# uci-cbcl/RP-Net

Measured on AMD Instinct MI355X. Metric: support/query pairs/sec (fwd+bwd, 1-shot 256x256, T=5), higher is better.
Workload: dtype f32

## Files before the change

rpnet_amd/csrc/conv_split.hip:

```cpp
#include <algorithm>

#include "conv_epilogue.h"
#include "split_bf16.h"

namespace rpnet {

constexpr bool IGLP = true;

template <int NP>
__global__ __launch_bounds__(256) void split_bf16_kernel(const float* __restrict__ x, const float* __restrict__ scale,
                                                          const int mode, unsigned short* __restrict__ out,
                                                          const size_t n8, const FastDiv fC, const size_t plane_elems) {
    RPNET_PASS_PRIORITY();
    for (size_t i = (size_t)blockIdx.x * 256 + threadIdx.x; i < n8; i += (size_t)gridDim.x * 256) {
        const f32x4 a = *reinterpret_cast<const f32x4*>(x + i * 8);
        const f32x4 b = *reinterpret_cast<const f32x4*>(x + i * 8 + 4);
        float v[8] = {a[0], a[1], a[2], a[3], b[0], b[1], b[2], b[3]};
        if (mode) {
            float s = scale[fC.div((unsigned)i)];
            if (mode == 2) s = 1.f - s;
#pragma unroll
            for (int q = 0; q < 8; ++q) v[q] *= s;
        }
        u32x4 o[NP];
        split8<NP>(v, o);
// ... 64 lines not shown
    if ((tid & 63) == 0) red[tid >> 6] = m;
    __syncthreads();
    if (tid == 0) {
        m = fmaxf(fmaxf(red[0], red[1]), fmaxf(red[2], red[3]));
        if (b < cout) t[b] = pow2_scale(m);
        else {
            const int cin = b - cout;
            u[cin < split ? off0 + cin : off1 + (cin - split)] = pow2_scale(m);
        }
    }
}

constexpr int kPackMax = 24;
struct PackItems {
    rpnet_pack_item it[kPackMax];
};

__global__ __launch_bounds__(256) void weight_row_scale_kernel(const PackItems items) {
    const rpnet_pack_item& q = items.it[blockIdx.y];
    if ((int)blockIdx.x >= q.cout + q.cin) return;
    weight_row_scale_block(blockIdx.x, q.w, q.row_scale_wp, q.row_scale_wd, q.cout, q.cin, q.taps, q.cin_off0, q.cin_split, q.cin_off1);
}

template <int NP, bool GATHER>
__device__ __forceinline__ void pack_weight_split_block(float (*tile)[32][33], const int bx, const int by, const float* __restrict__ w,
                                                        unsigned short* __restrict__ wp, unsigned short* __restrict__ wd, int taps,
                                                        int Cin_g, int Cout, int cin_w, int off0, int split, int off1,
                                                        const float* __restrict__ t_row, const float* __restrict__ u_row) {
    const int t = threadIdx.x;
    const int ci0 = bx * 32, co0 = by * 32;
    const int ncin = GATHER ? 32 : min(32, cin_w - ci0);
    if (GATHER) {
        for (int e = t; e < 32 * 32 * taps; e += 256) {
            const int col = e / (32 * taps), r = e - col * (32 * taps);
            const int c = r / taps, tap = r - c * taps;
            const int R = ci0 + c;
            int src = -1;
            if (R >= off0 && R < off0 + split) src = R - off0;
            else if (R >= off1 && R < off1 + (cin_w - split)) src = split + (R - off1);
            tile[tap][c][col] = src >= 0 ? w[((size_t)(co0 + col) * cin_w + src) * taps + tap] : 0.f;
        }
    } else {
        const int nel = ncin * taps;
        for (int e = t; e < 32 * nel; e += 256) {
            const int col = e / nel, r = e - col * nel;
            const int c = r / taps, tap = r - c * taps;
            tile[tap][c][col] = w[((size_t)(co0 + col) * cin_w + ci0) * taps + r];
        }
    }
    __syncthreads();
    const size_t plane = (size_t)taps * Cin_g * Cout;
    for (int e = t; e < taps * 32 * 4; e += 256) {
        const int g = e & 3, cl = (e >> 2) & 31, tap = e >> 7;
        if (g * 8 < ncin) {
            const int cin = ci0 + g * 8;
            const int row = GATHER ? cin : (cin < split ? off0 + cin : off1 + (cin - split));
            float v[8];
#pragma unroll
            for (int q = 0; q < 8; ++q) v[q] = tile[tap][g * 8 + q][cl];
            if (NP <= 2) {
                const float inv = 1.f / t_row[co0 + cl];
#pragma unroll
                for (int q = 0; q < 8; ++q) v[q] *= inv;
            }
            u32x4 o[NP];
            split8<NP>(v, o);
            const size_t dst = (((size_t)tap * (Cin_g >> 5) + (row >> 5)) * Cout + co0 + cl) * 32 + (row & 31);
#pragma unroll
            for (int p = 0; p < NP; ++p) *reinterpret_cast<u32x4*>(wp + p * plane + dst) = o[p];
        }
    }
    if (wd) {
        for (int e = t; e < taps * 32 * 4; e += 256) {
            const int g = e & 3, c = (e >> 2) & 31, tap = e >> 7;
            if (c < ncin) {
                const int cin = ci0 + c;
                const int row = GATHER ? cin : (cin < split ? off0 + cin : off1 + (cin - split));
                float v[8];
#pragma unroll
                for (int q = 0; q < 8; ++q) v[q] = tile[tap][c][g * 8 + q];
                if (NP <= 2) {
                    const float inv = 1.f / u_row[row];
#pragma unroll
                    for (int q = 0; q < 8; ++q) v[q] *= inv;
                }
                u32x4 o[NP];
                split8<NP>(v, o);
                const int tf = taps - 1 - tap;
                const size_t dst = (((size_t)tf * (Cout >> 5) + (co0 >> 5)) * Cin_g + row) * 32 + g * 8;
#pragma unroll
                for (int p = 0; p < NP; ++p) *reinterpret_cast<u32x4*>(wd + p * plane + dst) = o[p];
            }
        }
    }
}

__host__ __device__ static inline bool pack_needs_gather(const rpnet_pack_item& q) {
    return (q.cin % 8) || (q.cin_off0 % 8) || (q.cin_split % 8) || (q.cin_off1 % 8);
}

template <int NP>
__global__ __launch_bounds__(256) void pack_weight_split_kernel(const PackItems items) {
    __shared__ float tile[9][32][33];
    const rpnet_pack_item& q = items.it[blockIdx.y];
    const bool gather = pack_needs_gather(q);
    const int tx = gather ? q.cin_pad / 32 : (q.cin + 31) / 32, ntiles = tx * (q.cout / 32);
    if ((int)blockIdx.x >= ntiles) return;
    if (gather)
        pack_weight_split_block<NP, true>(tile, blockIdx.x % tx, blockIdx.x / tx, q.w, (unsigned short*)q.wp, (unsigned short*)q.wd, q.taps,
                                          q.cin_pad, q.cout, q.cin, q.cin_off0, q.cin_split, q.cin_off1, q.row_scale_wp, q.row_scale_wd);
    else
        pack_weight_split_block<NP, false>(tile, blockIdx.x % tx, blockIdx.x / tx, q.w, (unsigned short*)q.wp, (unsigned short*)q.wd, q.taps,
                                           q.cin_pad, q.cout, q.cin, q.cin_off0, q.cin_split, q.cin_off1, q.row_scale_wp, q.row_scale_wd);
}

template <int WGM, int WM, int WN, int NP, bool DB>
__global__ __launch_bounds__(WGM * 128, (DB ? 1 : (WGM == 2 ? 2 : 1))) void conv_igemm_split_kernel(
    const rpnet_conv_desc d, const int M, const int Cin, const int Cout, const int tiles_n, const int ntiles) {
    constexpr int NT = WGM * 128;
    constexpr int BM = 32 * WGM * WM, BN = 64 * WN;
    constexpr int RP = NT / 4;
    constexpr int AJ = BM / RP, BJ = (BN + RP - 1) / RP;
    constexpr bool B_PART = BN < RP;
    constexpr int A_BYTES = BM * 64, B_BYTES = BN * 64;
    constexpr int STAGE = NP * (A_BYTES + B_BYTES);
    __shared__ __attribute__((aligned(16))) unsigned char smem[cmax((DB ? 2 : 1) * STAGE, epilogue_lds_bytes<WN, WGM>())];

    const int t = threadIdx.x;
    const int lane = t & 63, wv = t >> 6;
    const int li = lane & 31, h = lane >> 5;
    const int wm = wv >> 1, wn = wv & 1;

    const int tile = xcd_swizzle(blockIdx.x, ntiles);
    const int tm = tile / tiles_n, tn = tile - tm * tiles_n;
    const int m0 = tm * BM, n0 = tn * BN;

// ... 805 lines not shown
                      "pack_conv_weights_split: channel ranges exceed cin_pad (item %d)", i);
        pk.it[i] = q;
        max_rows = std::max(max_rows, q.cout + q.cin);
        max_tiles = std::max(max_tiles, (pack_needs_gather(q) ? q.cin_pad / 32 : cdiv(q.cin, 32)) * (q.cout / 32));
    }
    for (int i = n; i < kPackMax; ++i) pk.it[i] = items[0];
    hipStream_t s = (hipStream_t)stream;
    if (planes <= 2)
        hipLaunchKernelGGL(weight_row_scale_kernel, dim3(max_rows, n), dim3(256), 0, s, pk);
    if (planes == 3) hipLaunchKernelGGL(pack_weight_split_kernel<3>, dim3(max_tiles, n), dim3(256), 0, s, pk);
    else if (planes == 2) hipLaunchKernelGGL(pack_weight_split_kernel<2>, dim3(max_tiles, n), dim3(256), 0, s, pk);
    else hipLaunchKernelGGL(pack_weight_split_kernel<1>, dim3(max_tiles, n), dim3(256), 0, s, pk);
    return check_launch("pack_conv_weights_split");
}

extern "C" int rpnet_pack_conv_weight_split(const float* w, void* wp, void* wd, int cout, int cin, int taps, int cin_off0,
                                            int cin_split, int cin_off1, int cin_pad, int planes, float* row_scale_wp,
                                            float* row_scale_wd, rpnet_stream_t stream) {
    rpnet_pack_item q;
    q.w = w; q.wp = wp; q.wd = wd; q.row_scale_wp = row_scale_wp; q.row_scale_wd = row_scale_wd;
    q.cout = cout; q.cin = cin; q.taps = taps; q.cin_off0 = cin_off0; q.cin_split = cin_split; q.cin_off1 = cin_off1; q.cin_pad = cin_pad;
    return rpnet_pack_conv_weights_split(&q, 1, planes, stream);
}
```

rpnet_amd/csrc/conv_up4_dma.hip:

```cpp
#include <type_traits>

#include "conv_epilogue.h"
#include "lds_dma.h"
#include "split_bf16.h"

namespace rpnet {

template <int N, int I = 0, typename F>
__device__ __forceinline__ void static_for_u(F&& f) {
    if constexpr (I < N) {
        f(std::integral_constant<int, I>{});
        static_for_u<N, I + 1>(f);
    }
}

template <int N>
__device__ __forceinline__ void wait_vmcnt() {
    static_assert(N >= 0 && N < 64, "vmcnt is a 6-bit counter");
    asm volatile("s_waitcnt vmcnt(%0)" ::"n"(N) : "memory");
}

template <int TW>
struct PatchRowsUp {
    static constexpr bool kAlwaysValid = true;
// ... 225 lines not shown
    asm volatile("s_waitcnt vmcnt(0)" ::: "memory");
    __builtin_amdgcn_s_barrier();

    if constexpr (DG) {
        conv_epilogue<WM, WN, 2, PatchRows<TW>, false>(d, acc, PatchRows<TW>{(n * Hl + y0) * Wl + x0, Wl}, d.N * Hl * Wl, Ncols, Hl * Wl, n0, tm,
                                                        wm, wn, li, h, smem);
    } else {
        conv_epilogue<WM, WN, 2, PatchRowsUp<TW>, false>(d, acc, PatchRowsUp<TW>{(n * H + 2 * y0 + fpy) * W + 2 * x0 + fpx, 2 * W}, d.N * H * W,
                                                          Cout_out, H * W, n0 - fphase * Cout_out, tm * 4 + fphase, wm, wn, li, h, smem,
                                                          fphase * Cout_out);
    }
}

__global__ __launch_bounds__(256) void upconv_collapse_kernel(const float* __restrict__ w, float* __restrict__ wc, const int Cout, const int Cin) {
    const size_t i = (size_t)blockIdx.x * 256 + threadIdx.x;
    if (i >= (size_t)4 * Cout * Cin) return;
    const int ci = (int)(i % Cin);
    const int co = (int)((i / Cin) % Cout), ph = (int)(i / ((size_t)Cin * Cout));
    const int py = ph >> 1, px = ph & 1;
    float k[9];
#pragma unroll
    for (int q = 0; q < 9; ++q) k[q] = w[((size_t)co * Cin + ci) * 9 + q];
    float o[4];
#pragma unroll
    for (int r = 0; r < 2; ++r)
#pragma unroll
        for (int c = 0; c < 2; ++c) {
            const int ya = r == 0 ? 0 : (py ? 2 : 1), yb = r == 0 ? (py ? 1 : 0) : 2;
            const int xa = c == 0 ? 0 : (px ? 2 : 1), xb = c == 0 ? (px ? 1 : 0) : 2;
            float s = 0.f;
            for (int ky = ya; ky <= yb; ++ky)
                for (int kx = xa; kx <= xb; ++kx) s += k[ky * 3 + kx];
            o[r * 2 + c] = s;
        }
    *reinterpret_cast<f32x4*>(wc + i * 4) = f32x4{o[0], o[1], o[2], o[3]};
}

static int up4_tw(int Hl, int Wl) {
    if (Wl % 32 == 0 && Hl % 8 == 0) return 32;
    if (Wl % 16 == 0 && Hl % 16 == 0) return 16;
    return 0;
}

static int up4_plan(const rpnet_conv_desc* d, int mode, int* tw, int* Kc, int* Ncols) {
    if (!d || (d->split_planes != 2 && d->split_planes != 1) || d->H % 2 || d->W % 2 || d->C1 || d->Co1 || d->x1 || d->y1) return 0;
    const int Hl = d->H / 2, Wl = d->W / 2;
    const bool one = d->split_planes == 1;
    *tw = up4_tw(Hl, Wl);
    if (!*tw || d->C0 % (one ? 64 : 32) || d->Co0 % (one ? 128 : 64)) return 0;
    *Kc = mode == 1 ? d->C0 : 4 * d->C0;
    *Ncols = mode == 1 ? 4 * d->Co0 : d->Co0;
    const size_t lim = (size_t)1 << 31;
    const size_t src = (size_t)d->N * (mode == 1 ? Hl * Wl : d->H * d->W) * d->C0 * 2 * d->split_planes;
    if (src >= lim || (size_t)2 * 4 * *Kc * *Ncols * 2 >= lim || (size_t)d->N * d->H * d->W >= lim) return 0;
    const long tiles_m = (long)d->N * Hl * Wl / 256;
    if (mode == 1) return (d->Co0 % 128 == 0) ? 2 : 1;
    if (one) return 2;
// ... 54 lines not shown
```

rpnet_amd/csrc/split_bf16.h:

```cpp
#pragma once
#include "common.h"

namespace rpnet {

using bf16x8 = __attribute__((ext_vector_type(8))) __bf16;
using u32x4 = __attribute__((ext_vector_type(4))) unsigned;
using u32x2 = __attribute__((ext_vector_type(2))) unsigned;

__device__ __forceinline__ unsigned bf16_bits(float x) {
    return (unsigned)__builtin_bit_cast(unsigned short, (__bf16)x);
}
__device__ __forceinline__ float bf16_val(unsigned b) { return __uint_as_float(b << 16); }

__device__ __forceinline__ unsigned f16_bits(float x) {
    return (unsigned)__builtin_bit_cast(unsigned short, (_Float16)x);
}
__device__ __forceinline__ float f16_val(unsigned b) {
    return (float)__builtin_bit_cast(_Float16, (unsigned short)b);
}

__device__ __forceinline__ float pow2_scale(float b) {
    const unsigned u = __float_as_uint(fmaxf(b, 0.f));
    int e = (int)((u >> 23) & 255u) - 127 + ((u & 0x7fffffu) ? 1 : 0);
    e = e - 15;
    e = e < -100 ? -100 : (e > 100 ? 100 : e);
    return __uint_as_float((unsigned)(e + 127) << 23);
}

template <int NP>
__device__ __forceinline__ void split8(const float (&v)[8], u32x4 (&out)[NP]) {
    unsigned hb[8], mb[8], lb[8];
#pragma unroll
    for (int q = 0; q < 8; ++q) {
        if (NP <= 2) {
            hb[q] = f16_bits(v[q]);
            if (NP == 2) mb[q] = f16_bits(v[q] - f16_val(hb[q]));
            continue;
        }
        hb[q] = bf16_bits(v[q]);
        const float r1 = v[q] - bf16_val(hb[q]);
        mb[q] = bf16_bits(r1);
        if (NP > 2) lb[q] = bf16_bits(r1 - bf16_val(mb[q]));
    }
#pragma unroll
    for (int q = 0; q < 4; ++q) {
        out[0][q] = hb[2 * q] | (hb[2 * q + 1] << 16);
        if (NP > 1) out[NP > 1 ? 1 : 0][q] = mb[2 * q] | (mb[2 * q + 1] << 16);
        if (NP > 2) out[NP - 1][q] = lb[2 * q] | (lb[2 * q + 1] << 16);
    }
// ... 21 lines not shown
```

rpnet_amd/functional.py:

```python
import collections
import contextlib
import ctypes as C
import os

import torch
from torch.autograd import Function
from torch.autograd.function import once_differentiable

from . import hip
from .hip import ConvDesc, call, ptr, query

BN_EPS = 1e-5
BN_MOMENTUM = 0.1

_ASYNC = {"on": False, "side": {}, "pending": set(), "queued": False, "fifo": [], "keep": []}

_MODES = {"f32": (0, False, 0), "bf16x3": (3, False, 0), "f16x2": (3, True, 2), "f16": (3, True, 1)}
_CORR_PRED_PLANES = True
_MATH = {}


def set_conv_math(mode):
    _MATH["mode"] = mode
    _MATH["planes"], _MATH["f16"], _MATH["f16_planes"] = _MODES[mode]
# ... 484 lines not shown
        if self._wp is None:
            self._pack_f32()
        return self._wd

    def split_packs(self, planes):
        pk = self.wps.get(planes) if self.wps else None
        if pk is None:
            w = self._weight
            pk = self.alloc_split(planes)
            call("rpnet_pack_conv_weight_split", ptr(w), ptr(pk[0]), ptr(pk[1]), self.cout, self.cin, self.taps,
                 self.off0, self.split, self.off1, self.cin_pad, planes, ptr(pk[2]) if planes <= 2 else None,
                 ptr(pk[3]) if planes <= 2 else None)
        return pk

    def up4_packs(self, planes):
        up = getattr(self, "_up4", None)
        if up is None:
            up = self._up4 = {}
        pk = up.get(planes)
        if pk is None:
            w = self._weight
            wc = torch.empty((4 * self.cout, self.cin, 2, 2), device=w.device, dtype=torch.float32)
            call("rpnet_upconv_collapse_weights", ptr(w), ptr(wc), self.cout, self.cin)
            n = 4 * self.cin * 4 * self.cout
            wp4 = torch.empty((planes, n), device=w.device, dtype=torch.float16)
            wd4 = torch.empty((planes, n), device=w.device, dtype=torch.float16)
            t4 = torch.empty(4 * self.cout, device=w.device, dtype=torch.float32)
            u4 = torch.empty(self.cin, device=w.device, dtype=torch.float32)
            call("rpnet_pack_conv_weight_split", ptr(wc), ptr(wp4), ptr(wd4), 4 * self.cout, self.cin, 4, 0, self.cin, self.cin, self.cin,
                 planes, ptr(t4), ptr(u4))
            pk = up[planes] = (wp4, wd4, t4, u4)
        return pk

    def alloc_split(self, planes):
        if self.wps is None:
            self.wps = {}
        n = self.taps * self.cin_pad * self.cout
        padded = self.cin_pad != self.cin
        w = self._weight
        key = (w.data_ptr(), tuple(w.shape), planes, self.cin_pad, self.off0, self.split, self.off1, str(w.device))
        if padded and self._pool is not None and key in self._pool:
            pk = self._pool[key]
            self.wps[planes] = pk
            return pk
        mk = torch.zeros if padded else torch.empty
        dt = torch.bfloat16 if planes == 3 else torch.float16
        wps, wds = mk((planes, n), device=w.device, dtype=dt), mk((planes, n), device=w.device, dtype=dt)
        if planes == 3:
            pk = (wps, wds)
        else:
            t = torch.empty(self.cout, device=w.device, dtype=torch.float32)
            u = (torch.ones if padded else torch.empty)(self.cin_pad, device=w.device, dtype=torch.float32)
            pk = (wps, wds, t, u)
        if padded and self._pool is not None:
            self._pool[key] = pk
        self.wps[planes] = pk
        return pk


class WeightCache:

    def __init__(self):
        self._d = {}
        self._ready = None
        self._padded = {}

    def clear(self):
        self._d.clear()
        self._ready = None

    def prepack_async(self, weights, planes, device, up4=()):
        main = torch.cuda.current_stream(device)
        ps = _pack_stream(device)
        ps.wait_stream(main)
        self._ready = None
        with torch.cuda.stream(ps):
            self.prepack(weights, planes, up4)
            ev = torch.cuda.Event()
            ev.record(ps)
        self._ready = (ev, set(), torch.cuda.is_current_stream_capturing())

    def get(self, weight, split=None):
        if self._ready is not None and self._ready[2] and not torch.cuda.is_current_stream_capturing():
            self._ready = None
        if self._ready is not None:
            sid = hip.stream()
            if sid not in self._ready[1]:
                torch.cuda.current_stream(weight.device).wait_event(self._ready[0])
                self._ready[1].add(sid)
        key = (weight.data_ptr(), weight._version, None if split is None else tuple(split))
        pw = self._d.get(key)
        if pw is None:
            pw = PackedWeight(weight.detach(), split, self._padded)
            self._d[key] = pw
        return pw

    def prepack(self, weights, planes, up4=()):
        up4 = list(up4) if (_UP4 and planes in (1, 2)) else []
        if up4:
            skip = {id(w) for w in up4}
            weights = [w for w in weights if id(w) not in skip]
            for w in up4:
                self.get(w).up4_packs(planes)
        pws = [self.get(w) for w in weights]
        pws = [pw for pw in pws if pw.taps == 9 and pw.cin_pad == pw.cin and pw.cin % 32 == 0 and pw.cout % 32 == 0
               and not (pw.wps and planes in pw.wps)]
        for i in range(0, len(pws), hip.PACK_MAX):
            chunk = pws[i:i + hip.PACK_MAX]
            items = (hip.PackItem * len(chunk))()
            for it, pw in zip(items, chunk):
                bufs = pw.alloc_split(planes)
                it.w, it.wp, it.wd = ptr(pw._weight), ptr(bufs[0]), ptr(bufs[1])
                it.row_scale_wp, it.row_scale_wd = (ptr(bufs[2]), ptr(bufs[3])) if planes <= 2 else (None, None)
                it.cout, it.cin, it.taps = pw.cout, pw.cin, pw.taps
                it.cin_off0, it.cin_split, it.cin_off1, it.cin_pad = pw.off0, pw.split, pw.off1, pw.cin_pad
            call("rpnet_pack_conv_weights_split", items, len(chunk), planes)

    def materialize(self, weights, planes):
        for w in weights:
            pw = self.get(w)
            if planes and pw.taps == 9 and pw.cin_pad == pw.cin and pw.cin % 32 == 0 and pw.cout % 32 == 0:
# ... 1101 lines not shown
```

rpnet_amd/hip.py:

```python
import ctypes as C
import os

import torch

_LIB_PATH = os.environ.get("RPNET_LIB_PATH") or os.path.join(os.path.dirname(os.path.abspath(__file__)), "librpnet_hip.so")
_lib = None

vp, ci, cf, cs, cd = C.c_void_p, C.c_int, C.c_float, C.c_size_t, C.c_double


class ConvDesc(C.Structure):
    _fields_ = [("x0", vp), ("x1", vp), ("C0", ci), ("C1", ci), ("w", vp), ("bias", vp), ("in_scale", vp),
                ("in_scale_mode", ci), ("y0", vp), ("y1", vp), ("Co0", ci), ("Co1", ci), ("ep_scale", vp),
                ("ep_shift", vp), ("ep_relu", ci), ("out_scale", vp), ("out_scale_mode", ci), ("accumulate", ci),
                ("N", ci), ("H", ci), ("W", ci), ("taps", ci), ("upsample", ci), ("groups", ci), ("dilation", ci), ("stats_partial", vp), ("split_planes", ci), ("y_split", vp), ("split_out_planes", ci),
                ("acc_scale_col", vp), ("acc_scale_x", vp), ("acc_scale_dy", vp), ("bnb_y", vp), ("bnb_stats", vp), ("bnb_partial", vp), ("bnb_pmax", vp), ("bnb_groups", ci),
                ("acc_scale_x1", vp), ("out_absmax", vp), ("tune", ci), ("y_split_scale", vp), ("splitk_ws", vp), ("splitk_ws_bytes", cs),
                ("skip_mask", vp), ("skip_mode", ci), ("skip_halo", ci), ("skip_ws", vp), ("tile_skip", vp),
                ("y_enc", vp), ("y_enc_stride", ci)]


PACK_MAX = 24


# ... 127 lines not shown
    "rpnet_adam_step_guarded": (ci, [vp, C.c_int64, vp, vp, vp, vp, vp, vp, vp, vp]),
}
GUARD_ABI_SYMBOLS = tuple(_GUARD_SIGS)
GUARD_ABI_VERSION = 1

_SURFACE_SIGS = {
    "rpnet_surface_abi_version": (ci, []),
    "rpnet_surface_workspace_bytes": (cs, [ci, ci, ci]),
    "rpnet_surface_tally": (ci, [vp, ci, vp, ci, ci, ci, ci, ci, vp, C.c_int64, vp, C.c_int64, C.c_int64, vp, cs, vp]),
}
SURFACE_ABI_SYMBOLS = tuple(_SURFACE_SIGS)
SURFACE_ABI_VERSION = 1

_CC_SIGS = {
    "rpnet_cc_abi_version": (ci, []),
    "rpnet_cc_workspace_bytes": (cs, [ci, ci, ci]),
    "rpnet_cc_label": (ci, [vp, ci, ci, ci, ci, ci, ci, vp, vp, C.c_int64, C.c_int64, vp, cs, vp]),
    "rpnet_cc_keep_largest": (ci, [vp, ci, vp, ci, ci, ci, ci, ci, vp, ci, vp, C.c_int64, vp, C.c_int64, C.c_int64, vp, cs, vp]),
}
CC_ABI_SYMBOLS = tuple(_CC_SIGS)
CC_ABI_VERSION = 1


def lib_path():
    return _LIB_PATH


def load():
    global _lib
    if _lib is None:
        if not os.path.exists(_LIB_PATH):
            raise RuntimeError(f"{_LIB_PATH} not found: build it with `make -C rpnet_amd/csrc` "
                               "(or __graft_entry__.build()); rpnet_amd has no CPU fallback")
        lib = C.CDLL(_LIB_PATH)
        lib.rpnet_version.restype = ci
        if lib.rpnet_version() != ABI_VERSION:
            raise RuntimeError(f"{_LIB_PATH} has ABI version {lib.rpnet_version()}, this binding was written for {ABI_VERSION} "
                               "(include/rpnet_abi.h RPNET_ABI_VERSION): rebuild it with `make -C rpnet_amd/csrc`")
        for name, (res, args) in (list(_SIGS.items()) + list(_EVAL_SIGS.items()) + list(_OPTIM_SIGS.items()) + list(_GUARD_SIGS.items())
                                  + list(_SURFACE_SIGS.items()) + list(_CC_SIGS.items())):
            fn = getattr(lib, name, None)
            if fn is None:
                raise RuntimeError(f"{_LIB_PATH} does not export {name}: rebuild it with `make -C rpnet_amd/csrc`")
            fn.restype, fn.argtypes = res, args
        if lib.rpnet_eval_abi_version() != EVAL_ABI_VERSION:
            raise RuntimeError(f"{_LIB_PATH} has evaluation-item ABI version {lib.rpnet_eval_abi_version()}, this binding was written for "
                               f"{EVAL_ABI_VERSION} (include/rpnet_eval_abi.h): rebuild it with `make -C rpnet_amd/csrc`")
        if lib.rpnet_optim_abi_version() != OPTIM_ABI_VERSION:
            raise RuntimeError(f"{_LIB_PATH} has optimizer ABI version {lib.rpnet_optim_abi_version()}, this binding was written for "
                               f"{OPTIM_ABI_VERSION} (include/rpnet_optim_abi.h): rebuild it with `make -C rpnet_amd/csrc`")
        if lib.rpnet_guard_abi_version() != GUARD_ABI_VERSION:
            raise RuntimeError(f"{_LIB_PATH} has gradient-guard ABI version {lib.rpnet_guard_abi_version()}, this binding was written for "
                               f"{GUARD_ABI_VERSION} (include/rpnet_guard_abi.h): rebuild it with `make -C rpnet_amd/csrc`")
        if lib.rpnet_surface_abi_version() != SURFACE_ABI_VERSION:
            raise RuntimeError(f"{_LIB_PATH} has surface-distance ABI version {lib.rpnet_surface_abi_version()}, this binding was written "
                               f"for {SURFACE_ABI_VERSION} (include/rpnet_surface_abi.h): rebuild it with `make -C rpnet_amd/csrc`")
        if lib.rpnet_cc_abi_version() != CC_ABI_VERSION:
            raise RuntimeError(f"{_LIB_PATH} has connected-component ABI version {lib.rpnet_cc_abi_version()}, this binding was written "
                               f"for {CC_ABI_VERSION} (include/rpnet_cc_abi.h): rebuild it with `make -C rpnet_amd/csrc`")
        _lib = lib
    return _lib


def ptr(t):
    return None if t is None else t.data_ptr()


try:
    _raw_stream, _cur_device = torch._C._cuda_getCurrentRawStream, torch._C._cuda_getDevice
except AttributeError:
    _raw_stream = None


def stream():
    if _raw_stream is not None:
        return _raw_stream(_cur_device())
    return torch.cuda.current_stream().cuda_stream


def call(name, *args):
    lib = load()
    rc = getattr(lib, name)(*args, stream())
# ... 14 lines not shown
```

rpnet_amd/modules.py:

```python
import itertools
import os

import torch
import torch.nn as nn

from . import functional as RF
from .schedule import Schedule

_FANIN = 2
_PREPACK = True
_ZSKIP = True
_F16_MIN_PIXELS = int(os.environ.get("RPNET_F16_MIN_PIXELS", "262144"))
_F16_MIN_PIXELS_EVAL = int(os.environ.get("RPNET_F16_MIN_PIXELS_EVAL", "524288"))
_CRE_STREAMS = True
_CRE_STREAMS_MAX_PIXELS = 16384
_CRE_STREAMS_TRAIN = os.environ.get("RPNET_CRE_STREAMS_TRAIN", "1") == "1"
_ENC_STREAMS = int(os.environ.get("RPNET_ENC_STREAMS", "1"))
_NET_SERIAL = itertools.count(1)


def _to_nhwc(x):
    return x.permute(0, 2, 3, 1).contiguous()


# ... 352 lines not shown
        if repack:
            cache.clear()

        supp = (supp_imgs[0][0] if n_ways * n_shots == 1 else torch.cat([torch.cat(way, 0) for way in supp_imgs], 0)).float()
        qry = qry_imgs[0].float()
        RF.hip.require_gpu(supp, qry)
        ns = supp.shape[0]
        f16_min, f16_min_eval = sch.get("f16_min_pixels", _F16_MIN_PIXELS), sch.get("f16_min_pixels_eval", _F16_MIN_PIXELS_EVAL)
        thr = f16_min if (self.training or not f16_min_eval or not f16_min or RF._EVAL_PREDICT) else f16_min_eval
        RF.set_f16_active((ns + B) * H * W >= thr)
        pred_key = None
        if RF.f16_mode():
            RF.reset_absmax_pool(supp.device)
            if not self.training and not torch.is_grad_enabled() and RF._EVAL_PREDICT:
                pred_key = (self._serial, RF.conv_math(), ns, B, H, W, self.num_iter, n_ways, n_shots, self.forced_masks is not None)
                RF.pred_begin(supp.device, pred_key, allow=not getattr(self, "_pred_redo", False))
        planes = RF.pack_planes()
        if _PREPACK and planes and repack:
            ups = ()
            if self.training or RF.f16_mode():
                enc_n = (ns + B,) if ns == B else (ns, B)
                ups = tuple(m.up[1].weight for m, f in ((self.encoder.Up5, 8), (self.encoder.Up4, 4))
                            if RF.up4_layer_ok(m.up[1].weight, planes, [(n, H // f, W // f) for n in enc_n + ((ns, B) if ns == B else ())]))
            if self.training and supp.is_cuda:
                cache.prepack_async(self._pack_weights(), planes, supp.device, ups)
            else:
                cache.prepack(self._pack_weights(), planes, ups)
        enc_mask = fore_mask[0][0].float() if self.encoder.mask_feature_map else None
        if enc_mask is not None and ns != B:
            raise NotImplementedError("mask_feature_map with more than one support image per episode: the reference "
                                      "concatenates B masks onto Wa*Sh*B images (net/unet.py:438) and fails")
        enc_streams, fanin = sch.get("enc_streams", _ENC_STREAMS), sch.get("fanin", _FANIN)
        two_chains = (self.training and supp.is_cuda and enc_mask is None and
                      (enc_streams == 2 or (enc_streams == 1 and ns != B and ns <= 2 * B)))
        RF.order_begin(two_chains)
        split_fan = False
        if ns == B and not two_chains:
            d4 = self.encoder.forward_nhwc(torch.cat([supp, qry], 0).reshape(ns + B, H, W, 1), cache, groups=2,
                                           mask=None if enc_mask is None else torch.cat([enc_mask, enc_mask], 0))
            s_supp = s_qry = d4.scale
            d4 = d4.x
            split_fan = d4.requires_grad and fanin >= 2 and n_ways * n_shots == 1
            if split_fan:
                uses = RF.SplitFan.apply(d4, ns, 2, 2 * self.num_iter)
                supp_d4, qry_d4, fan_supp, fan_qry = uses[0], uses[2], uses[:2], uses[2:]
            else:
                supp_d4, qry_d4 = RF.SplitRows.apply(d4, ns) if (d4.requires_grad and fanin) else (d4[:ns], d4[ns:])
        elif two_chains:
            main, side = torch.cuda.current_stream(supp.device), RF._cre_stream(supp.device)
            qin = qry.reshape(B, H, W, 1)
# ... 153 lines not shown
```

Baseline: 486.1.

## Fuse per-layer weight packing into one table-driven two-kernel launch

Replaces the per-layer weight row-scale and split-pack launches with a precomputed device tile table covering every layer, including collapsed up-convolutions and the padded correlation layer. Two kernels run over it: one computes row and column maxima with atomics into double-buffered scratch, the other packs and publishes the scales. The goal is to cut the many small kernel launches and host calls made each training step during prepack. It also adds a vectorized quad load for 9-tap tiles. In exchange it brings a new ABI, plan caching keyed on weight pointers, and ping-pong scale buffers whose correctness depends on kernel ordering.

```diff
diff --git a/include/rpnet_pack_abi.h b/include/rpnet_pack_abi.h
--- /dev/null
+++ b/include/rpnet_pack_abi.h
@@ -0,0 +1,41 @@
+#ifndef RPNET_PACK_ABI_H
+#define RPNET_PACK_ABI_H
+
+#include <stddef.h>
+#include <stdint.h>
+
+#include "rpnet_abi.h"
+
+#ifdef __cplusplus
+extern "C" {
+#endif
+
+#define RPNET_PACK_ABI_VERSION 1
+int rpnet_pack_abi_version(void);
+
+struct rpnet_pack_layer {
+    rpnet_pack_item item;
+    float* maxima;
+    int32_t collapse;
+    int32_t reserved;
+};
+
+struct rpnet_pack_tile {
+    int32_t layer;
+    uint16_t bx, by;
+};
+
+struct rpnet_pack_head {
+    int32_t n_layers, n_tiles;
+    uint32_t set_scale;
+    uint32_t set_pack;
+};
+
+size_t rpnet_pack_plan_bytes(const struct rpnet_pack_layer* layers, int n);
+int rpnet_pack_plan(const struct rpnet_pack_layer* layers, int n, int planes, void* table, size_t table_bytes, int* n_tiles);
+int rpnet_pack_fused(void* table, int n_layers, int n_tiles, int planes, rpnet_stream_t stream);
+
+#ifdef __cplusplus
+}
+#endif
+#endif
diff --git a/rpnet_amd/csrc/conv_split.hip b/rpnet_amd/csrc/conv_split.hip
--- a/rpnet_amd/csrc/conv_split.hip
+++ b/rpnet_amd/csrc/conv_split.hip
@@ -1,6 +1,7 @@
 #include <algorithm>
 
 #include "conv_epilogue.h"
+#include "rpnet_pack_abi.h"
 #include "split_bf16.h"
 
 namespace rpnet {
@@ -111,14 +112,22 @@
     weight_row_scale_block(blockIdx.x, q.w, q.row_scale_wp, q.row_scale_wd, q.cout, q.cin, q.taps, q.cin_off0, q.cin_split, q.cin_off1);
 }
 
-template <int NP, bool GATHER>
-__device__ __forceinline__ void pack_weight_split_block(float (*tile)[32][33], const int bx, const int by, const float* __restrict__ w,
-                                                        unsigned short* __restrict__ wp, unsigned short* __restrict__ wd, int taps,
-                                                        int Cin_g, int Cout, int cin_w, int off0, int split, int off1,
-                                                        const float* __restrict__ t_row, const float* __restrict__ u_row) {
+template <bool GATHER, bool QUADS = false>
+__device__ __forceinline__ int pack_tile_load(float (*tile)[32][33], const int ci0, const int co0, const float* __restrict__ w, int taps,
+                                              int cin_w, int off0, int split, int off1) {
     const int t = threadIdx.x;
-    const int ci0 = bx * 32, co0 = by * 32;
     const int ncin = GATHER ? 32 : min(32, cin_w - ci0);
+    if (QUADS && !GATHER && taps == 9 && ncin == 32 && cin_w % 4 == 0 && (reinterpret_cast<size_t>(w) & 15) == 0) {
+#pragma unroll
+        for (int j = 0; j < 9; ++j) {
+            const int e = t + 256 * j;
+            const int col = e / 72, r = (e - col * 72) * 4;
+            const f32x4 v = *reinterpret_cast<const f32x4*>(w + ((size_t)(co0 + col) * cin_w + ci0) * 9 + r);
+#pragma unroll
+            for (int i = 0; i < 4; ++i) tile[(r + i) % 9][(r + i) / 9][col] = v[i];
+        }
+        return ncin;
+    }
     if (GATHER) {
         for (int e = t; e < 32 * 32 * taps; e += 256) {
             const int col = e / (32 * taps), r = e - col * (32 * taps);
@@ -137,18 +146,30 @@
             tile[tap][c][col] = w[((size_t)(co0 + col) * cin_w + ci0) * taps + r];
         }
     }
-    __syncthreads();
+    return ncin;
+}
+
+template <bool GATHER>
+__device__ __forceinline__ int pack_row(const int cin, int off0, int split, int off1) {
+    return GATHER ? cin : (cin < split ? off0 + cin : off1 + (cin - split));
+}
+
+template <int NP, bool GATHER, bool FROM_MAX = false>
+__device__ __forceinline__ void pack_tile_store(float (*tile)[32][33], const int ci0, const int co0, const int ncin,
+                                                unsigned short* __restrict__ wp, unsigned short* __restrict__ wd, int taps, int Cin_g,
+                                                int Cout, int off0, int split, int off1, const float* __restrict__ t_row,
+                                                const float* __restrict__ u_row) {
+    const int t = threadIdx.x;
     const size_t plane = (size_t)taps * Cin_g * Cout;
     for (int e = t; e < taps * 32 * 4; e += 256) {
         const int g = e & 3, cl = (e >> 2) & 31, tap = e >> 7;
         if (g * 8 < ncin) {
-            const int cin = ci0 + g * 8;
-            const int row = GATHER ? cin : (cin < split ? off0 + cin : off1 + (cin - split));
+            const int row = pack_row<GATHER>(ci0 + g * 8, off0, split, off1);
             float v[8];
 #pragma unroll
             for (int q = 0; q < 8; ++q) v[q] = tile[tap][g * 8 + q][cl];
             if (NP <= 2) {
-                const float inv = 1.f / t_row[co0 + cl];
+                const float inv = 1.f / (FROM_MAX ? pow2_scale(t_row[co0 + cl]) : t_row[co0 + cl]);
 #pragma unroll
                 for (int q = 0; q < 8; ++q) v[q] *= inv;
             }
@@ -163,13 +184,12 @@
         for (int e = t; e < taps * 32 * 4; e += 256) {
             const int g = e & 3, c = (e >> 2) & 31, tap = e >> 7;
             if (c < ncin) {
-                const int cin = ci0 + c;
-                const int row = GATHER ? cin : (cin < split ? off0 + cin : off1 + (cin - split));
+                const int row = pack_row<GATHER>(ci0 + c, off0, split, off1);
                 float v[8];
 #pragma unroll
                 for (int q = 0; q < 8; ++q) v[q] = tile[tap][c][g * 8 + q];
                 if (NP <= 2) {
-                    const float inv = 1.f / u_row[row];
+                    const float inv = 1.f / (FROM_MAX ? pow2_scale(u_row[row]) : u_row[row]);
 #pragma unroll
                     for (int q = 0; q < 8; ++q) v[q] *= inv;
                 }
@@ -182,6 +202,16 @@
             }
         }
     }
+}
+
+template <int NP, bool GATHER>
+__device__ __forceinline__ void pack_weight_split_block(float (*tile)[32][33], const int bx, const int by, const float* __restrict__ w,
+                                                        unsigned short* __restrict__ wp, unsigned short* __restrict__ wd, int taps,
+                                                        int Cin_g, int Cout, int cin_w, int off0, int split, int off1,
+                                                        const float* __restrict__ t_row, const float* __restrict__ u_row) {
+    const int ncin = pack_tile_load<GATHER>(tile, bx * 32, by * 32, w, taps, cin_w, off0, split, off1);
+    __syncthreads();
+    pack_tile_store<NP, GATHER>(tile, bx * 32, by * 32, ncin, wp, wd, taps, Cin_g, Cout, off0, split, off1, t_row, u_row);
 }
 
 __host__ __device__ static inline bool pack_needs_gather(const rpnet_pack_item& q) {
@@ -201,6 +231,161 @@
     else
         pack_weight_split_block<NP, false>(tile, blockIdx.x % tx, blockIdx.x / tx, q.w, (unsigned short*)q.wp, (unsigned short*)q.wd, q.taps,
                                            q.cin_pad, q.cout, q.cin, q.cin_off0, q.cin_split, q.cin_off1, q.row_scale_wp, q.row_scale_wd);
+}
+
+struct PackWork {
+    const rpnet_pack_layer* L;
+    int bx, by;
+};
+__device__ __forceinline__ PackWork pack_work(const void* table) {
+    const rpnet_pack_head* h = (const rpnet_pack_head*)table;
+    const rpnet_pack_layer* layers = (const rpnet_pack_layer*)(h + 1);
+    const rpnet_pack_tile tl = ((const rpnet_pack_tile*)(layers + h->n_layers))[blockIdx.x];
+    return PackWork{layers + tl.layer, (int)tl.bx, (int)tl.by};
+}
+
+__device__ __forceinline__ void collapse_tile_load(float (&k)[4][9], const int ci0, const int co0, const float* __restrict__ w, int cin_w) {
+#pragma unroll
+    for (int j = 0; j < 4; ++j) {
+        const int pr = threadIdx.x + 256 * j, col = pr >> 5, c = pr & 31;
+        const float* src = w + ((size_t)(co0 + col) * cin_w + ci0 + c) * 9;
+#pragma unroll
+        for (int q = 0; q < 9; ++q) k[j][q] = src[q];
+    }
+}
+__device__ __forceinline__ void collapse_tile_phase(float (*tile)[32][33], const float (&k)[4][9], const int ph) {
+#pragma unroll
+    for (int j = 0; j < 4; ++j) {
+        const int pr = threadIdx.x + 256 * j, col = pr >> 5, c = pr & 31;
+        float o[4];
+        upconv_collapse_taps(k[j], ph >> 1, ph & 1, o);
+#pragma unroll
+        for (int q = 0; q < 4; ++q) tile[q][c][col] = o[q];
+    }
+}
+
+__device__ __forceinline__ void pack_tile_maxima(float (*tile)[32][33], unsigned* smax, const int taps, const int ncin) {
+    const int t = threadIdx.x;
+    if (t < 64) smax[t] = 0u;
+    __syncthreads();
+    const int idx = t & 31, part = (t >> 5) & 3;
+    float m = 0.f;
+    if (t < 128) {
+        for (int tap = 0; tap < taps; ++tap)
+            for (int c = part; c < ncin; c += 4) m = fmaxf(m, fabsf(tile[tap][c][idx]));
+    } else if (idx < ncin) {
+        for (int j = part; j < taps * 32; j += 4) m = fmaxf(m, fabsf(tile[j >> 5][idx][j & 31]));
+    }
+    atomicMax(&smax[(t < 128 ? 0 : 32) + idx], __float_as_uint(m));
+    __syncthreads();
+}
+
+template <bool GATHER>
+__device__ __forceinline__ void pack_maxima_merge(const unsigned* smax, float* mx, const rpnet_pack_item& q, const int ci0, const int row0,
+                                                  const int ncin) {
+    const int t = threadIdx.x;
+    if (t < 32) atomicMax((unsigned*)mx + row0 + t, smax[t]);
+    else if (t < 64 && t - 32 < ncin) {
+        const int cin = ci0 + t - 32;
+        const bool real = !GATHER || (cin >= q.cin_off0 && cin < q.cin_off0 + q.cin_split) ||
+                          (cin >= q.cin_off1 && cin < q.cin_off1 + (q.cin - q.cin_split));
+        if (real) atomicMax((unsigned*)mx + q.cout + pack_row<GATHER>(cin, q.cin_off0, q.cin_split, q.cin_off1), smax[t]);
+    }
+}
+
+__global__ __launch_bounds__(256) void pack_fused_scale_kernel(void* table) {
+    __shared__ float tile[9][32][33];
+    __shared__ unsigned smax[64];
+    rpnet_pack_head* h = (rpnet_pack_head*)table;
+    const unsigned set = h->set_scale & 1u;
+    if (blockIdx.x == 0 && threadIdx.x == 0) h->set_pack = set ^ 1u;
+    const PackWork k = pack_work(table);
+    const rpnet_pack_item& q = k.L->item;
+    float* mx = k.L->maxima + (size_t)set * (q.cout + q.cin_pad);
+    const int ci0 = k.bx * 32, co0 = k.by * 32;
+    if (k.L->collapse) {
+        float k9[4][9];
+        collapse_tile_load(k9, ci0, co0, q.w, q.cin);
+        for (int ph = 0; ph < 4; ++ph) {
+            if (ph) __syncthreads();
+            collapse_tile_phase(tile, k9, ph);
+            pack_tile_maxima(tile, smax, 4, 32);
+            pack_maxima_merge<false>(smax, mx, q, ci0, ph * (q.cout >> 2) + co0, 32);
+        }
+    } else if (pack_needs_gather(q)) {
+        const int ncin = pack_tile_load<true>(tile, ci0, co0, q.w, q.taps, q.cin, q.cin_off0, q.cin_split, q.cin_off1);
+        pack_tile_maxima(tile, smax, q.taps, ncin);
+        pack_maxima_merge<true>(smax, mx, q, ci0, co0, ncin);
+    } else {
+        const int ncin = pack_tile_load<false, true>(tile, ci0, co0, q.w, q.taps, q.cin, q.cin_off0, q.cin_split, q.cin_off1);
+        pack_tile_maxima(tile, smax, q.taps, ncin);
+        pack_maxima_merge<false>(smax, mx, q, ci0, co0, ncin);
+    }
+}
+
+template <bool GATHER>
+__device__ __forceinline__ void pack_scales_publish(const rpnet_pack_item& q, const float* mx, float* other, const int bx, const int ci0,
+                                                    const int row0, const bool cols) {
+    const int t = threadIdx.x;
+    if (bx == 0 && t < 32) {
+        q.row_scale_wp[row0 + t] = pow2_scale(mx[row0 + t]);
+        other[row0 + t] = 0.f;
+    }
+    if (cols && t >= 32 && t < 64) {
+        const int cin = ci0 + t - 32;
+        const bool real = GATHER ? ((cin >= q.cin_off0 && cin < q.cin_off0 + q.cin_split) ||
+                                    (cin >= q.cin_off1 && cin < q.cin_off1 + (q.cin - q.cin_split)))
+                                 : cin < q.cin;
+        if (real) {
+            const int row = pack_row<GATHER>(cin, q.cin_off0, q.cin_split, q.cin_off1);
+            q.row_scale_wd[row] = pow2_scale(mx[q.cout + row]);
+            other[q.cout + row] = 0.f;
+        }
+    }
+}
+
+template <int NP>
+__global__ __launch_bounds__(256) void pack_fused_kernel(void* table) {
+    __shared__ float tile[9][32][33];
+    constexpr bool F16 = NP <= 2;
+    rpnet_pack_head* h = (rpnet_pack_head*)table;
+    const PackWork k = pack_work(table);
+    const rpnet_pack_item& q = k.L->item;
+    const float* mx = nullptr;
+    float* other = nullptr;
+    if (F16) {
+        const unsigned clr = h->set_pack & 1u;
+        if (blockIdx.x == 0 && threadIdx.x == 0) h->set_scale = clr;
+        mx = k.L->maxima + (size_t)(clr ^ 1u) * (q.cout + q.cin_pad);
+        other = k.L->maxima + (size_t)clr * (q.cout + q.cin_pad);
+    }
+    const int ci0 = k.bx * 32, co0 = k.by * 32;
+    unsigned short* wp = (unsigned short*)q.wp;
+    unsigned short* wd = (unsigned short*)q.wd;
+    if (k.L->collapse) {
+        float k9[4][9];
+        collapse_tile_load(k9, ci0, co0, q.w, q.cin);
+        for (int ph = 0; ph < 4; ++ph) {
+            const int row0 = ph * (q.cout >> 2) + co0;
+            if (ph) __syncthreads();
+            collapse_tile_phase(tile, k9, ph);
+            __syncthreads();
+            pack_tile_store<NP, false, true>(tile, ci0, row0, 32, wp, wd, 4, q.cin_pad, q.cout, 0, q.cin, q.cin, mx, mx + q.cout);
+            if (F16) pack_scales_publish<false>(q, mx, other, k.bx, ci0, row0, k.by == 0 && ph == 0);
+        }
+    } else if (pack_needs_gather(q)) {
+        const int ncin = pack_tile_load<true>(tile, ci0, co0, q.w, q.taps, q.cin, q.cin_off0, q.cin_split, q.cin_off1);
+        __syncthreads();
+        pack_tile_store<NP, true, true>(tile, ci0, co0, ncin, wp, wd, q.taps, q.cin_pad, q.cout, q.cin_off0, q.cin_split, q.cin_off1, mx,
+                                        mx + q.cout);
+        if (F16) pack_scales_publish<true>(q, mx, other, k.bx, ci0, co0, k.by == 0);
+    } else {
+        const int ncin = pack_tile_load<false, true>(tile, ci0, co0, q.w, q.taps, q.cin, q.cin_off0, q.cin_split, q.cin_off1);
+        __syncthreads();
+        pack_tile_store<NP, false, true>(tile, ci0, co0, ncin, wp, wd, q.taps, q.cin_pad, q.cout, q.cin_off0, q.cin_split, q.cin_off1, mx,
+                                         mx + q.cout);
+        if (F16) pack_scales_publish<false>(q, mx, other, k.bx, ci0, co0, k.by == 0);
+    }
 }
 
 template <int WGM, int WM, int WN, int NP, bool DB>
@@ -1052,3 +1237,83 @@
     q.cout = cout; q.cin = cin; q.taps = taps; q.cin_off0 = cin_off0; q.cin_split = cin_split; q.cin_off1 = cin_off1; q.cin_pad = cin_pad;
     return rpnet_pack_conv_weights_split(&q, 1, planes, stream);
 }
+
+extern "C" int rpnet_pack_abi_version(void) { return RPNET_PACK_ABI_VERSION; }
+
+namespace rpnet {
+static int pack_layer_tiles(const rpnet_pack_layer& l, int* tx, int* ty) {
+    const rpnet_pack_item& q = l.item;
+    *tx = l.collapse ? q.cin / 32 : (pack_needs_gather(q) ? q.cin_pad / 32 : cdiv(q.cin, 32));
+    *ty = (l.collapse ? q.cout / 4 : q.cout) / 32;
+    return *tx * *ty;
+}
+
+static int pack_plan_check(const rpnet_pack_layer* layers, int n, int planes, long* tiles) {
+    RPNET_REQUIRE(layers && n >= 1, RPNET_ERR_ARG, "pack_plan: %d layers", n);
+    RPNET_REQUIRE(planes >= 0 && planes <= 3, RPNET_ERR_SHAPE, "pack_plan: planes %d", planes);
+    *tiles = 0;
+    for (int i = 0; i < n; ++i) {
+        const rpnet_pack_item& q = layers[i].item;
+        RPNET_REQUIRE(q.w && q.wp, RPNET_ERR_ARG, "pack_plan: null pointer (layer %d)", i);
+        RPNET_REQUIRE(planes == 0 || planes == 3 || (q.row_scale_wp && q.row_scale_wd && layers[i].maxima), RPNET_ERR_ARG,
+                      "pack_plan: fp16 planes (1 or 2) need the row scale outputs and the maxima (layer %d)", i);
+        RPNET_REQUIRE(q.cout > 0 && q.cin > 0 && q.cout % 32 == 0 && q.cin_pad > 0 && q.cin_pad % 32 == 0 &&
+                          (q.taps == 9 || q.taps == 1 || q.taps == 4),
+                      RPNET_ERR_SHAPE, "pack_plan: cout %d cin %d cin_pad %d taps %d (layer %d)", q.cout, q.cin, q.cin_pad, q.taps, i);
+        RPNET_REQUIRE(q.cin_off0 >= 0 && q.cin_off1 >= 0 && q.cin_split >= 0 && q.cin_split <= q.cin &&
+                          q.cin_off0 + q.cin_split <= q.cin_pad && q.cin_off1 + (q.cin - q.cin_split) <= q.cin_pad,
+                      RPNET_ERR_SHAPE, "pack_plan: channel ranges exceed cin_pad (layer %d)", i);
+        if (layers[i].collapse)
+            RPNET_REQUIRE(q.taps == 4 && q.cout % 128 == 0 && q.cin % 32 == 0 && q.cin_off0 == 0 && q.cin_split == q.cin &&
+                              q.cin_off1 == q.cin && q.cin_pad == q.cin,
+                          RPNET_ERR_SHAPE, "pack_plan: collapsed layer %d: cout %d cin %d taps %d, or channel ranges", i, q.cout, q.cin, q.taps);
+        int tx, ty;
+        *tiles += pack_layer_tiles(layers[i], &tx, &ty);
+        RPNET_REQUIRE(tx <= 65535 && ty <= 65535 && *tiles < (1l << 30), RPNET_ERR_SHAPE, "pack_plan: too many tiles (layer %d)", i);
+    }
+    return RPNET_OK;
+}
+}
+
+extern "C" size_t rpnet_pack_plan_bytes(const rpnet_pack_layer* layers, int n) {
+    long tiles = 0;
+    if (rpnet::pack_plan_check(layers, n, 0, &tiles) != RPNET_OK) return 0;
+    return sizeof(rpnet_pack_head) + (size_t)n * sizeof(rpnet_pack_layer) + (size_t)tiles * sizeof(rpnet_pack_tile);
+}
+
+extern "C" int rpnet_pack_plan(const rpnet_pack_layer* layers, int n, int planes, void* table, size_t table_bytes, int* n_tiles) {
+    using namespace rpnet;
+    RPNET_REQUIRE(table && n_tiles, RPNET_ERR_ARG, "pack_plan: null pointer");
+    RPNET_REQUIRE(planes >= 1, RPNET_ERR_SHAPE, "pack_plan: planes %d", planes);
+    long tiles = 0;
+    const int rc = pack_plan_check(layers, n, planes, &tiles);
+    if (rc != RPNET_OK) return rc;
+    const size_t need = sizeof(rpnet_pack_head) + (size_t)n * sizeof(rpnet_pack_layer) + (size_t)tiles * sizeof(rpnet_pack_tile);
+    RPNET_REQUIRE(table_bytes >= need, RPNET_ERR_WORKSPACE, "pack_plan: table of %zu bytes, %zu needed", table_bytes, need);
+    rpnet_pack_head* h = (rpnet_pack_head*)table;
+    *h = rpnet_pack_head{n, (int)tiles, 0u, 1u};
+    rpnet_pack_layer* L = (rpnet_pack_layer*)(h + 1);
+    rpnet_pack_tile* T = (rpnet_pack_tile*)(L + n);
+    for (int i = 0; i < n; ++i) {
+        L[i] = layers[i];
+        L[i].reserved = 0;
+        int tx, ty;
+        pack_layer_tiles(layers[i], &tx, &ty);
+        for (int by = 0; by < ty; ++by)
+            for (int bx = 0; bx < tx; ++bx) *T++ = rpnet_pack_tile{i, (uint16_t)bx, (uint16_t)by};
+    }
+    *n_tiles = (int)tiles;
+    return RPNET_OK;
+}
+
+extern "C" int rpnet_pack_fused(void* table, int n_layers, int n_tiles, int planes, rpnet_stream_t stream) {
+    using namespace rpnet;
+    RPNET_REQUIRE(table && n_layers >= 1 && n_tiles >= 1, RPNET_ERR_ARG, "pack_fused: table %p, %d layers, %d tiles", table, n_layers, n_tiles);
+    RPNET_REQUIRE(planes >= 1 && planes <= 3, RPNET_ERR_SHAPE, "pack_fused: planes %d", planes);
+    hipStream_t s = (hipStream_t)stream;
+    if (planes <= 2) hipLaunchKernelGGL(pack_fused_scale_kernel, dim3(n_tiles), dim3(256), 0, s, table);
+    if (planes == 3) hipLaunchKernelGGL(pack_fused_kernel<3>, dim3(n_tiles), dim3(256), 0, s, table);
+    else if (planes == 2) hipLaunchKernelGGL(pack_fused_kernel<2>, dim3(n_tiles), dim3(256), 0, s, table);
+    else hipLaunchKernelGGL(pack_fused_kernel<1>, dim3(n_tiles), dim3(256), 0, s, table);
+    return check_launch("pack_fused");
+}
diff --git a/rpnet_amd/csrc/conv_up4_dma.hip b/rpnet_amd/csrc/conv_up4_dma.hip
--- a/rpnet_amd/csrc/conv_up4_dma.hip
+++ b/rpnet_amd/csrc/conv_up4_dma.hip
@@ -271,17 +271,7 @@
 #pragma unroll
     for (int q = 0; q < 9; ++q) k[q] = w[((size_t)co * Cin + ci) * 9 + q];
     float o[4];
-#pragma unroll
-    for (int r = 0; r < 2; ++r)
-#pragma unroll
-        for (int c = 0; c < 2; ++c) {
-            const int ya = r == 0 ? 0 : (py ? 2 : 1), yb = r == 0 ? (py ? 1 : 0) : 2;
-            const int xa = c == 0 ? 0 : (px ? 2 : 1), xb = c == 0 ? (px ? 1 : 0) : 2;
-            float s = 0.f;
-            for (int ky = ya; ky <= yb; ++ky)
-                for (int kx = xa; kx <= xb; ++kx) s += k[ky * 3 + kx];
-            o[r * 2 + c] = s;
-        }
+    upconv_collapse_taps(k, py, px, o);
     *reinterpret_cast<f32x4*>(wc + i * 4) = f32x4{o[0], o[1], o[2], o[3]};
 }
 
diff --git a/rpnet_amd/csrc/split_bf16.h b/rpnet_amd/csrc/split_bf16.h
--- a/rpnet_amd/csrc/split_bf16.h
+++ b/rpnet_amd/csrc/split_bf16.h
@@ -25,6 +25,20 @@
     e = e - 15;
     e = e < -100 ? -100 : (e > 100 ? 100 : e);
     return __uint_as_float((unsigned)(e + 127) << 23);
+}
+
+__device__ __forceinline__ void upconv_collapse_taps(const float (&k)[9], const int py, const int px, float (&o)[4]) {
+#pragma unroll
+    for (int r = 0; r < 2; ++r)
+#pragma unroll
+        for (int c = 0; c < 2; ++c) {
+            const int ya = r == 0 ? 0 : (py ? 2 : 1), yb = r == 0 ? (py ? 1 : 0) : 2;
+            const int xa = c == 0 ? 0 : (px ? 2 : 1), xb = c == 0 ? (px ? 1 : 0) : 2;
+            float s = 0.f;
+            for (int ky = ya; ky <= yb; ++ky)
+                for (int kx = xa; kx <= xb; ++kx) s += k[ky * 3 + kx];
+            o[r * 2 + c] = s;
+        }
 }
 
 template <int NP>
diff --git a/rpnet_amd/functional.py b/rpnet_amd/functional.py
--- a/rpnet_amd/functional.py
+++ b/rpnet_amd/functional.py
@@ -530,15 +530,16 @@
             w = self._weight
             wc = torch.empty((4 * self.cout, self.cin, 2, 2), device=w.device, dtype=torch.float32)
             call("rpnet_upconv_collapse_weights", ptr(w), ptr(wc), self.cout, self.cin)
-            n = 4 * self.cin * 4 * self.cout
-            wp4 = torch.empty((planes, n), device=w.device, dtype=torch.float16)
-            wd4 = torch.empty((planes, n), device=w.device, dtype=torch.float16)
-            t4 = torch.empty(4 * self.cout, device=w.device, dtype=torch.float32)
-            u4 = torch.empty(self.cin, device=w.device, dtype=torch.float32)
-            call("rpnet_pack_conv_weight_split", ptr(wc), ptr(wp4), ptr(wd4), 4 * self.cout, self.cin, 4, 0, self.cin, self.cin, self.cin,
-                 planes, ptr(t4), ptr(u4))
-            pk = up[planes] = (wp4, wd4, t4, u4)
+            pk = up[planes] = self.alloc_up4(planes)
+            call("rpnet_pack_conv_weight_split", ptr(wc), ptr(pk[0]), ptr(pk[1]), 4 * self.cout, self.cin, 4, 0, self.cin, self.cin, self.cin,
+                 planes, ptr(pk[2]), ptr(pk[3]))
         return pk
+
+    def alloc_up4(self, planes):
+        w = self._weight
+        n = 4 * self.cin * 4 * self.cout
+        return (torch.empty((planes, n), device=w.device, dtype=torch.float16), torch.empty((planes, n), device=w.device, dtype=torch.float16),
+                torch.empty(4 * self.cout, device=w.device, dtype=torch.float32), torch.empty(self.cin, device=w.device, dtype=torch.float32))
 
     def alloc_split(self, planes):
         if self.wps is None:
@@ -566,24 +567,67 @@
         return pk
 
 
+_FUSED_PACK = True
+
+
+class FusedPack:
+
+    def __init__(self, layers, planes):
+        self.planes = planes
+        self.bufs = [pw.alloc_up4(planes) if collapse else pw.alloc_split(planes) for pw, collapse in layers]
+        dev = layers[0][0]._weight.device
+        rows = [(4 * pw.cout if collapse else pw.cout) + pw.cin_pad for pw, collapse in layers]
+        self.maxima = torch.zeros(2 * sum(rows), device=dev, dtype=torch.float32) if planes <= 2 else None
+        items = (hip.PackLayer * len(layers))()
+        at = 0
+        for it, (pw, collapse), pk, r in zip(items, layers, self.bufs, rows):
+            q = it.item
+            q.w, q.wp, q.wd = ptr(pw._weight), ptr(pk[0]), ptr(pk[1])
+            if planes <= 2:
+                q.row_scale_wp, q.row_scale_wd, it.maxima = ptr(pk[2]), ptr(pk[3]), self.maxima.data_ptr() + 4 * at
+                at += 2 * r
+            q.cout, q.cin, q.taps = (4 * pw.cout, pw.cin, 4) if collapse else (pw.cout, pw.cin, pw.taps)
+            q.cin_off0, q.cin_split, q.cin_off1, q.cin_pad = pw.off0, pw.split, pw.off1, pw.cin_pad
+            it.collapse = 1 if collapse else 0
+        nbytes = hip.query("rpnet_pack_plan_bytes", items, len(layers))
+        host = torch.zeros(max(nbytes, 8), dtype=torch.uint8)
+        n_tiles = C.c_int(0)
+        rc = hip.query("rpnet_pack_plan", items, len(layers), planes, host.data_ptr(), nbytes, C.byref(n_tiles))
+        if rc != 0 or nbytes == 0:
+            raise RuntimeError(f"rpnet_pack_plan failed (rc={rc}): {hip.load().rpnet_last_error_string().decode()}")
+        self.table = host.to(dev)
+        self.n_layers, self.n_tiles = len(layers), n_tiles.value
+
+    def adopt(self, layers):
+        for (pw, collapse), pk in zip(layers, self.bufs):
+            if collapse:
+                pw._up4 = {self.planes: pk}
+            else:
+                pw.wps = {self.planes: pk}
+
+    def run(self):
+        call("rpnet_pack_fused", ptr(self.table), self.n_layers, self.n_tiles, self.planes)
+
+
 class WeightCache:
 
     def __init__(self):
         self._d = {}
         self._ready = None
         self._padded = {}
+        self._fused = {}
 
     def clear(self):
         self._d.clear()
         self._ready = None
 
-    def prepack_async(self, weights, planes, device, up4=()):
+    def prepack_async(self, weights, planes, device, up4=(), padded=()):
         main = torch.cuda.current_stream(device)
         ps = _pack_stream(device)
         ps.wait_stream(main)
         self._ready = None
         with torch.cuda.stream(ps):
-            self.prepack(weights, planes, up4)
+            self.prepack(weights, planes, up4, padded)
             ev = torch.cuda.Event()
             ev.record(ps)
         self._ready = (ev, set(), torch.cuda.is_current_stream_capturing())
@@ -603,8 +647,25 @@
             self._d[key] = pw
         return pw
 
-    def prepack(self, weights, planes, up4=()):
+    def prepack(self, weights, planes, up4=(), padded=()):
         up4 = list(up4) if (_UP4 and planes in (1, 2)) else []
+        if _FUSED_PACK:
+            ups = {id(w) for w in up4}
+            layers = [(self.get(w), id(w) in ups) for w in weights] + [(self.get(w, split), False) for w, split in padded]
+            layers = [(pw, c) for pw, c in layers if pw.cout % 32 == 0 and (
+                (pw.taps == 9 and pw.cin_pad == pw.cin and pw.cin % 32 == 0) or (pw.taps == 1 and pw.cin_pad != pw.cin and pw.cin_pad % 32 == 0))]
+            if not layers:
+                return
+            key = (planes,) + tuple((pw._weight.data_ptr(), pw.cout, pw.cin, pw.taps, pw.off0, pw.split, pw.off1, pw.cin_pad, c,
+                                     str(pw._weight.device)) for pw, c in layers)
+            fp = self._fused.get(key)
+            if fp is None:
+                if len(self._fused) >= 2:
+                    self._fused.pop(next(iter(self._fused)))
+                fp = self._fused[key] = FusedPack(layers, planes)
+            fp.adopt(layers)
+            fp.run()
+            return
         if up4:
             skip = {id(w) for w in up4}
             weights = [w for w in weights if id(w) not in skip]
diff --git a/rpnet_amd/hip.py b/rpnet_amd/hip.py
--- a/rpnet_amd/hip.py
+++ b/rpnet_amd/hip.py
@@ -173,6 +173,21 @@
 CC_ABI_VERSION = 1
 
 
+
+class PackLayer(C.Structure):
+    _fields_ = [("item", PackItem), ("maxima", vp), ("collapse", C.c_int32), ("reserved", C.c_int32)]
+
+
+_PACK_SIGS = {
+    "rpnet_pack_abi_version": (ci, []),
+    "rpnet_pack_plan_bytes": (cs, [C.POINTER(PackLayer), ci]),
+    "rpnet_pack_plan": (ci, [C.POINTER(PackLayer), ci, ci, vp, cs, C.POINTER(ci)]),
+    "rpnet_pack_fused": (ci, [vp, ci, ci, ci, vp]),
+}
+PACK_ABI_SYMBOLS = tuple(_PACK_SIGS)
+PACK_ABI_VERSION = 1
+
+
 def lib_path():
     return _LIB_PATH
 
@@ -189,7 +204,7 @@
             raise RuntimeError(f"{_LIB_PATH} has ABI version {lib.rpnet_version()}, this binding was written for {ABI_VERSION} "
                                "(include/rpnet_abi.h RPNET_ABI_VERSION): rebuild it with `make -C rpnet_amd/csrc`")
         for name, (res, args) in (list(_SIGS.items()) + list(_EVAL_SIGS.items()) + list(_OPTIM_SIGS.items()) + list(_GUARD_SIGS.items())
-                                  + list(_SURFACE_SIGS.items()) + list(_CC_SIGS.items())):
+                                  + list(_SURFACE_SIGS.items()) + list(_CC_SIGS.items()) + list(_PACK_SIGS.items())):
             fn = getattr(lib, name, None)
             if fn is None:
                 raise RuntimeError(f"{_LIB_PATH} does not export {name}: rebuild it with `make -C rpnet_amd/csrc`")
@@ -209,6 +224,9 @@
         if lib.rpnet_cc_abi_version() != CC_ABI_VERSION:
             raise RuntimeError(f"{_LIB_PATH} has connected-component ABI version {lib.rpnet_cc_abi_version()}, this binding was written "
                                f"for {CC_ABI_VERSION} (include/rpnet_cc_abi.h): rebuild it with `make -C rpnet_amd/csrc`")
+        if lib.rpnet_pack_abi_version() != PACK_ABI_VERSION:
+            raise RuntimeError(f"{_LIB_PATH} has weight-pack ABI version {lib.rpnet_pack_abi_version()}, this binding was written for "
+                               f"{PACK_ABI_VERSION} (include/rpnet_pack_abi.h): rebuild it with `make -C rpnet_amd/csrc`")
         _lib = lib
     return _lib
 
diff --git a/rpnet_amd/modules.py b/rpnet_amd/modules.py
--- a/rpnet_amd/modules.py
+++ b/rpnet_amd/modules.py
@@ -398,10 +398,12 @@
                 enc_n = (ns + B,) if ns == B else (ns, B)
                 ups = tuple(m.up[1].weight for m, f in ((self.encoder.Up5, 8), (self.encoder.Up4, 4))
                             if RF.up4_layer_ok(m.up[1].weight, planes, [(n, H // f, W // f) for n in enc_n + ((ns, B) if ns == B else ())]))
+            kk = (2 * self.cre.radius + 1) ** 2
+            padded = ((self.cre.q[0].weight, (kk, RF.corr_stride(self.cre.radius))),)
             if self.training and supp.is_cuda:
-                cache.prepack_async(self._pack_weights(), planes, supp.device, ups)
+                cache.prepack_async(self._pack_weights(), planes, supp.device, ups, padded)
             else:
-                cache.prepack(self._pack_weights(), planes, ups)
+                cache.prepack(self._pack_weights(), planes, ups, padded)
         enc_mask = fore_mask[0][0].float() if self.encoder.mask_feature_map else None
         if enc_mask is not None and ns != B:
             raise NotImplementedError("mask_feature_map with more than one support image per episode: the reference "
```

After: 487.6, median of 5. No clear change (+0.3%).
